# prismformore/Multi-Task-Transformer

Hardware: AMD Instinct MI355X
Metric: training images/sec (512x512, 6 tasks) (higher is better)
Workload: dtype f32(bf16x3)

## Files before the change

include/mtt_hip.h:

```cpp
#ifndef MTT_HIP_H
#define MTT_HIP_H

#include <stddef.h>
#include <stdint.h>

#ifdef __cplusplus
extern "C" {
#endif

#define MTT_ABI_VERSION 14

enum { MTT_F32 = 0, MTT_BF16 = 1, MTT_SPLIT = 2 };
enum { MTT_PREC_BF16 = 0, MTT_PREC_X3 = 1 };
enum { MTT_E_BADARG = -1, MTT_E_ALIGN = -2, MTT_E_UNSUPPORTED = -3 };

enum {
  MTT_OP_K = 0,
  MTT_OP_R = 1,
  MTT_OP_CONV_K = 2,
  MTT_OP_CONV_R = 3
};
enum { MTT_ACT_NONE = 0, MTT_ACT_GELU = 1, MTT_ACT_RELU = 2, MTT_ACT_GELU_BWD = 3, MTT_ACT_RELU_BWD = 4,
       MTT_ACT_GELU_DAUX = 5 ,
       MTT_ACT_MUL_AUX = 6    };
enum { MTT_STORE_ROWS = 0, MTT_STORE_PIXSHUF2 = 1 };
enum { MTT_GEMM_AUTO = 0,
       MTT_GEMM_GENERAL = 1           ,
       MTT_GEMM_DMA256 = 3            ,
       MTT_GEMM_DMA128 = 4            ,
       MTT_GEMM_GENERAL_EPILOGUE = 11  };
enum { MTT_ATTN_AUTO = 0, MTT_ATTN_PLAIN = 1,
       MTT_ATTN_FAST_V0 = 2 ,
       MTT_ATTN_FAST_V1 = 3  };

typedef struct {
  int32_t H, W;
  int32_t C;
  int32_t Cp;
  int32_t dil;
  int32_t flip;
} mtt_conv_geom;

typedef struct {
  const void* A; const void* B; void* D;
  int32_t M, N, K;
  int32_t a_op, b_op;
  int32_t a_dtype, b_dtype, d_dtype;
  int32_t prec;
  int64_t lda, ldb, ldd;
  int32_t a_mb; int64_t a_bs;
  int32_t d_mb; int64_t d_bs;
  int32_t batch, batch_inner;
  int64_t a_zo, a_zi, b_zo, b_zi, d_zo, d_zi;
  mtt_conv_geom conv;
  float alpha;
  const float* colscale; const float* colshift; int64_t col_zo, col_zi;
  int32_t act;
  const void* aux_in; void* aux_out; int32_t aux_dtype; int64_t ldaux; int64_t aux_zo, aux_zi;
  const float* rowscale; int32_t n_prompt;
  const float* resid; int64_t ldr; int32_t r_mb; int64_t r_bs; int64_t r_zo, r_zi;
  int32_t n_store;
  int32_t store_mode;
  int32_t ps_H, ps_W, ps_Co;
  int32_t variant;
  const void* A_lo; const void* B_lo; void* D_lo;
  float* colsum_out; float* colsum_ws;
  const float* a_scale; const float* a_shift; int32_t a_act; void* a_aux16; int64_t ld_a16;
} mtt_gemm_desc;
size_t mtt_gemm_colsum_ws_floats(const mtt_gemm_desc* d);

int mtt_abi_version(void);
size_t mtt_desc_size(int which);
int mtt_gemm(const mtt_gemm_desc* d, void* stream);
int mtt_gemm_variant(const mtt_gemm_desc* d);

typedef struct {
  const void* qkv; void* out; float* rawlog; float* lse;
  int32_t B, N, nH, T;
  int32_t dtype, prec;
  float scale;
  int32_t variant;
  const void* qkv_lo; void* out_lo;
} mtt_attn_desc;
int mtt_attn_fwd(const mtt_attn_desc* d, void* stream);
int mtt_attn_bwd(const mtt_attn_desc* d, const void* dout, const float* drawlog, void* dqkv, float* stat, void* stream);

typedef struct {
  const void* S; void* P; const void* dP; void* dS; const float* extra;
  int64_t rows, cols, ld; int32_t s_dtype, p_dtype; float scale;
  int64_t rows_per_mat; int32_t extra_rows; int64_t extra_ld;
} mtt_softmax_desc;
int mtt_softmax_fwd(const mtt_softmax_desc* d, void* stream);
int mtt_softmax_bwd(const mtt_softmax_desc* d, void* stream);

typedef struct {
  const float* x; void* y; const float* gamma; const float* beta; float* mean; float* rstd;
  const void* dy; float* dx; float* dgamma; float* dbeta;
  int64_t rows; int32_t C; int64_t ldx, ldy; int32_t y_dtype; float eps;
  const float* dx_in;
  float* ws;
  void* y_lo;
  float* y32; int64_t ldy32;
} mtt_ln_desc;
size_t mtt_layernorm_bwd_ws_floats(int64_t rows, int32_t C);
int mtt_layernorm_fwd(const mtt_ln_desc* d, void* stream);
int mtt_layernorm_bwd(const mtt_ln_desc* d, void* stream);

int mtt_patchify16(const float* img, void* cols, int B, int H, int W, int out_dtype, void* stream);

typedef struct {
  const void* q; const void* xn; float* rawchan;
  int32_t B, T, N, C, h, w, nh, nw; int32_t dtype; int64_t ldq;
  float* ws;
  const void* xn_lo;
} mtt_chanlogit_desc;
size_t mtt_chan_logits_ws_floats(const mtt_chanlogit_desc* d);
// ... 237 lines not shown
```

multi-task-transformer_amd/_lib.py:

```python
import ctypes as C
import os

import torch

_HERE = os.path.dirname(os.path.abspath(__file__))
LIB_PATH = os.path.join(_HERE, "libmtt_hip.so")

ABI_VERSION = 14
F32, BF16, SPLIT = 0, 1, 2
PREC_BF16, PREC_X3 = 0, 1
OP_K, OP_R, OP_CONV_K, OP_CONV_R = 0, 1, 2, 3
ACT_NONE, ACT_GELU, ACT_RELU, ACT_GELU_BWD, ACT_RELU_BWD, ACT_GELU_DAUX, ACT_MUL_AUX = 0, 1, 2, 3, 4, 5, 6
STORE_ROWS, STORE_PIXSHUF2 = 0, 1
GEMM_AUTO, GEMM_GENERAL, GEMM_DMA256, GEMM_DMA128, GEMM_GENERAL_EPILOGUE = 0, 1, 3, 4, 11
ATTN_AUTO, ATTN_PLAIN = 0, 1

i32, i64, f32, ptr = C.c_int32, C.c_int64, C.c_float, C.c_void_p


class ConvGeom(C.Structure):
    _fields_ = [("H", i32), ("W", i32), ("C", i32), ("Cp", i32), ("dil", i32), ("flip", i32)]


class GemmDesc(C.Structure):
    _fields_ = [
        ("A", ptr), ("B", ptr), ("D", ptr),
        ("M", i32), ("N", i32), ("K", i32),
        ("a_op", i32), ("b_op", i32),
        ("a_dtype", i32), ("b_dtype", i32), ("d_dtype", i32),
        ("prec", i32),
        ("lda", i64), ("ldb", i64), ("ldd", i64),
        ("a_mb", i32), ("a_bs", i64),
        ("d_mb", i32), ("d_bs", i64),
        ("batch", i32), ("batch_inner", i32),
        ("a_zo", i64), ("a_zi", i64), ("b_zo", i64), ("b_zi", i64), ("d_zo", i64), ("d_zi", i64),
        ("conv", ConvGeom),
        ("alpha", f32),
        ("colscale", ptr), ("colshift", ptr), ("col_zo", i64), ("col_zi", i64),
        ("act", i32),
        ("aux_in", ptr), ("aux_out", ptr), ("aux_dtype", i32), ("ldaux", i64), ("aux_zo", i64), ("aux_zi", i64),
        ("rowscale", ptr), ("n_prompt", i32),
        ("resid", ptr), ("ldr", i64), ("r_mb", i32), ("r_bs", i64), ("r_zo", i64), ("r_zi", i64),
        ("n_store", i32), ("store_mode", i32),
        ("ps_H", i32), ("ps_W", i32), ("ps_Co", i32),
        ("variant", i32),
        ("A_lo", ptr), ("B_lo", ptr), ("D_lo", ptr),
        ("colsum_out", ptr), ("colsum_ws", ptr),
        ("a_scale", ptr), ("a_shift", ptr), ("a_act", i32), ("a_aux16", ptr), ("ld_a16", i64),
    ]


class AttnDesc(C.Structure):
    _fields_ = [("qkv", ptr), ("out", ptr), ("rawlog", ptr), ("lse", ptr),
                ("B", i32), ("N", i32), ("nH", i32), ("T", i32), ("dtype", i32), ("prec", i32), ("scale", f32),
                ("variant", i32), ("qkv_lo", ptr), ("out_lo", ptr)]


class SoftmaxDesc(C.Structure):
    _fields_ = [("S", ptr), ("P", ptr), ("dP", ptr), ("dS", ptr), ("extra", ptr),
                ("rows", i64), ("cols", i64), ("ld", i64), ("s_dtype", i32), ("p_dtype", i32), ("scale", f32),
                ("rows_per_mat", i64), ("extra_rows", i32), ("extra_ld", i64)]


class LnDesc(C.Structure):
    _fields_ = [("x", ptr), ("y", ptr), ("gamma", ptr), ("beta", ptr), ("mean", ptr), ("rstd", ptr),
                ("dy", ptr), ("dx", ptr), ("dgamma", ptr), ("dbeta", ptr),
                ("rows", i64), ("C", i32), ("ldx", i64), ("ldy", i64), ("y_dtype", i32), ("eps", f32), ("dx_in", ptr), ("ws", ptr),
                ("y_lo", ptr), ("y32", ptr), ("ldy32", i64)]


class ChanLogitDesc(C.Structure):
    _fields_ = [("q", ptr), ("xn", ptr), ("rawchan", ptr),
                ("B", i32), ("T", i32), ("N", i32), ("C", i32), ("h", i32), ("w", i32), ("nh", i32), ("nw", i32),
                ("dtype", i32), ("ldq", i64), ("ws", ptr), ("xn_lo", ptr)]


class ModulateDesc(C.Structure):
    _fields_ = [("x", ptr), ("x_ld", i64), ("x_bs", i64), ("rawlog", ptr), ("rawchan", ptr), ("out", ptr),
                ("B", i32), ("T", i32), ("N", i32), ("C", i32), ("h", i32), ("w", i32), ("nh", i32), ("nw", i32),
                ("out_dtype", i32), ("hg", i32), ("out_lo", ptr)]


class CtrDesc(C.Structure):
    _fields_ = [("fea", ptr), ("out", ptr), ("wmix", ptr), ("T", i32), ("B", i32), ("rows_per_b", i64), ("ld", i64),
                ("C", i32), ("fea_dtype", i32), ("accumulate", i32), ("out_dtype", i32)]


class ResizeDesc(C.Structure):
    _fields_ = [("in_", ptr), ("out", ptr), ("B", i32), ("C", i32), ("Hin", i32), ("Win", i32), ("Hout", i32), ("Wout", i32),
                ("ld_in", i64), ("ld_out", i64), ("in_dtype", i32), ("out_dtype", i32), ("out_nchw", i32), ("accumulate", i32)]


class BnDesc(C.Structure):
    _fields_ = [("x", ptr), ("y", ptr), ("dy", ptr), ("dx", ptr),
                ("mean_out", ptr), ("m2_out", ptr), ("mean", ptr), ("rstd", ptr), ("gamma", ptr), ("beta", ptr),
                ("dsum", ptr), ("dsumxh", ptr),
                ("rows", i64), ("C", i32), ("ld", i64), ("dtype", i32), ("act", i32),
                ("Z", i32), ("x_zs", i64), ("p_zs", i64), ("g_dtype", i32)]
# ... 295 lines not shown
```

multi-task-transformer_amd/csrc/attn_bwd.hip:

```cpp
#include "mtt_device.h"
#include <type_traits>

namespace {

constexpr int HD = 64;
constexpr int KTILE = 64 * HD * 2;
constexpr float LOG2E = 1.4426950408889634f;

struct BwdP {
  const bf16_t* qkv; const bf16_t* dout; const float* stat; const float* drawlog; bf16_t* dqkv;
  int B, N, nH, T, Np; float scale;
};

__global__ __launch_bounds__(256) void attn_stat_kernel(const bf16_t* out, const bf16_t* dout, const float* lse, float* stat, int B, int N,
                                                        int nH, int Np) {
  const int C8 = nH * 8;
  const int64_t total = (int64_t)B * N * C8;
  const int64_t t = (int64_t)blockIdx.x * 256 + threadIdx.x;
  float s = 0.f;
  if (t < total) {
    const u32x4 a = *(const u32x4*)(out + t * 8), g = *(const u32x4*)(dout + t * 8);
#pragma unroll
    for (int j = 0; j < 4; ++j) s += lo_of(a[j]) * lo_of(g[j]) + hi_of(a[j]) * hi_of(g[j]);
  }
  s += __shfl_xor(s, 1, 64); s += __shfl_xor(s, 2, 64); s += __shfl_xor(s, 4, 64);
  if (t < total && (threadIdx.x & 7) == 0) {
    const int64_t tok = t / C8;
    const int h = (int)(t % C8) >> 3;
    const int b = (int)(tok / N), n = (int)(tok % N);
    float* row = stat + ((int64_t)b * nH + h) * 2 * Np;
    row[n] = s;
    row[Np + n] = lse[((int64_t)b * nH + h) * N + n] * LOG2E;
    if (n == N - 1)
      for (int k = N; k < Np; ++k) { row[k] = 0.f; row[Np + k] = 0.f; }
  }
}

MTT_DEV u32x4 perm_frag(const unsigned char* tile, int row, int ks, int lg) {
  const u32x2 lo = *(const u32x2*)(tile + lds_off(row, 4 * ks + (lg >> 1)) + (lg & 1) * 8);
  const u32x2 hi = *(const u32x2*)(tile + lds_off(row, 4 * ks + 2 + (lg >> 1)) + (lg & 1) * 8);
  return (u32x4){lo[0], lo[1], hi[0], hi[1]};
}

template <bool TR>
MTT_DEV void store_units(unsigned char* rowmajor, unsigned char* transposed, const u32x4 (&sh)[4], int kq, int rb) {
#pragma unroll
  for (int i = 0; i < 4; ++i) *(u32x4*)(rowmajor + lds_off(kq * 4 + i, rb)) = sh[i];
  if (TR) {
    u32x2 piece[8];
    transpose4x8(sh, piece);
#pragma unroll
    for (int j = 0; j < 8; ++j) *(u32x2*)(transposed + lds_off(rb * 8 + j, kq >> 1) + (kq & 1) * 8) = piece[j];
  }
}

__device__ __attribute__((aligned(32))) const unsigned g_bwd_zero_page[8] = {0u, 0u, 0u, 0u, 0u, 0u, 0u, 0u};
MTT_DEV int bwd_swz(int row) { return (((row >> 1) & 3) << 1) | ((row >> 3) & 1); }
MTT_DEV void bwd_glds16(const bf16_t* src, unsigned char* lds_wave_base) {
  __builtin_amdgcn_global_load_lds((const __attribute__((address_space(1))) void*)src,
                                   (__attribute__((address_space(3))) void*)lds_wave_base, 16, 0, 0);
}
template <int OFF>
MTT_DEV u32x2 bwd_ds_read_tr16(unsigned addr) {
  u32x2 r;
  asm volatile("ds_read_b64_tr_b16 %0, %1 offset:%2" : "=v"(r) : "v"(addr), "n"(OFF) : "memory");
  return r;
}
#define BWD_TRW(x) "+v"(x)
#define BWD_WAIT_TR8(a, b)                                                                                                              \
  asm volatile("s_waitcnt lgkmcnt(0)" : BWD_TRW(a[0]), BWD_TRW(a[1]), BWD_TRW(a[2]), BWD_TRW(a[3]), BWD_TRW(b[0]), BWD_TRW(b[1]), BWD_TRW(b[2]), BWD_TRW(b[3]) :: "memory")
#define BWD_WAIT_TR16(a, b, c, d)                                                                                                       \
  asm volatile("s_waitcnt lgkmcnt(0)" : BWD_TRW(a[0]), BWD_TRW(a[1]), BWD_TRW(a[2]), BWD_TRW(a[3]), BWD_TRW(b[0]), BWD_TRW(b[1]), BWD_TRW(b[2]), BWD_TRW(b[3]), \
               BWD_TRW(c[0]), BWD_TRW(c[1]), BWD_TRW(c[2]), BWD_TRW(c[3]), BWD_TRW(d[0]), BWD_TRW(d[1]), BWD_TRW(d[2]), BWD_TRW(d[3]) :: "memory")

template <int VER>
__global__ __launch_bounds__(256, 2) void attn_bwd_dq_kernel(const BwdP p) {
  extern __shared__ __attribute__((aligned(16))) unsigned char smem[];
  constexpr int STAGE = (VER == 2 ? 2 : 3) * KTILE;
  const int nqb = (p.N + 127) / 128;
  const int wi = xcd_remap(blockIdx.x, gridDim.x);
  const int qb = wi % nqb, bh_ = wi / nqb;
  const int h = bh_ % p.nH, b = bh_ / p.nH;
  const int N = p.N, C = p.nH * HD;
  const int tid = threadIdx.x, lane = tid & 63, wave = tid >> 6;
  const int li = lane & 15, lg = lane >> 4;
  const int64_t tok0 = (int64_t)b * N;
  const int64_t bh = (int64_t)b * p.nH + h;
  const int q0 = qb * 128 + wave * 32;
  const bool active = q0 < N;

  u32x4 qf[2][2], gf[2][2], dummy;
  float lse2[2], Dq[2];
#pragma unroll
  for (int sub = 0; sub < 2; ++sub) {
// ... 453 lines not shown
            const u32x4 ga = *(const u32x4*)(Gh + lds_off(qs * 16 + li, kh * 4 + lg));
#pragma unroll
            for (int kt = 0; kt < 2; ++kt) {
              s[q2][kt] = mfma16(qa, kf[kt][kh], s[q2][kt]);
              dp[q2][kt] = mfma16(ga, vf[kt][kh], dp[q2][kt]);
            }
          }
        }
        if (VER >= 1) __builtin_amdgcn_s_setprio(0);
        }
        u32x4 pb[2], dsb[2];
#pragma unroll
        for (int kt = 0; kt < 2; ++kt) {
          float pv[2][4], ds[2][4];
#pragma unroll
          for (int q2 = 0; q2 < 2; ++q2) {
            const float lr[4] = {L4[q2].x, L4[q2].y, L4[q2].z, L4[q2].w};
            const float dr[4] = {D4[q2].x, D4[q2].y, D4[q2].z, D4[q2].w};
#pragma unroll
            for (int r = 0; r < 4; ++r) {
              pv[q2][r] = __builtin_amdgcn_exp2f(fmaf(s[q2][kt][r], sc2, -lr[r]));
              if (!full && q0 + (2 * ks + q2) * 16 + lg * 4 + r >= N) pv[q2][r] = 0.f;
              ds[q2][r] = pv[q2][r] * (dp[q2][kt][r] - dr[r]);
            }
          }
          if (add_raw && ks == 0) {
            const int key = key0 + kt * 16 + li;
#pragma unroll
            for (int r = 0; r < 4; ++r) {
              const int q = lg * 4 + r;
              if (q < p.T && key < N) ds[0][r] += p.drawlog[(bh * p.T + q) * N + key] * inv_scale;
            }
          }
          pb[kt] = (u32x4){pack2(pv[0][0], pv[0][1]), pack2(pv[0][2], pv[0][3]), pack2(pv[1][0], pv[1][1]), pack2(pv[1][2], pv[1][3])};
          dsb[kt] = (u32x4){pack2(ds[0][0], ds[0][1]), pack2(ds[0][2], ds[0][3]), pack2(ds[1][0], ds[1][1]), pack2(ds[1][2], ds[1][3])};
        }
        if (VER >= 1) __builtin_amdgcn_s_setprio(1);
#pragma unroll
        for (int dt = 0; dt < 4; ++dt) {
          u32x4 ga, qa;
          if constexpr (VER == 2) {
            ga = (u32x4){gtl[dt][0], gtl[dt][1], gth[dt][0], gth[dt][1]};
            qa = (u32x4){qtl[dt][0], qtl[dt][1], qth[dt][0], qth[dt][1]};
          } else {
            ga = perm_frag(Gt, dt * 16 + li, ks, lg);
            qa = perm_frag(Qt, dt * 16 + li, ks, lg);
          }
#pragma unroll
          for (int kt = 0; kt < 2; ++kt) {
            dv[kt][dt] = mfma16(ga, pb[kt], dv[kt][dt]);
            dk[kt][dt] = mfma16(qa, dsb[kt], dk[kt][dt]);
          }
        }
        if (VER >= 1) __builtin_amdgcn_s_setprio(0);
      }
    }
    if (more) {
      if (VER == 2) asm volatile("s_waitcnt vmcnt(0)" ::: "memory");
      else stage_store(smem + (ST < 0 ? ((j + 1) & 1) : (1 - ST)) * STAGE);
    }
    __syncthreads();
  };
  if (VER >= 1) {
    for (int j = 0; j < nq; j += 2) {
      tile(std::integral_constant<int, 0>{}, j);
      if (j + 1 < nq) tile(std::integral_constant<int, 1>{}, j + 1);
    }
  } else {
    for (int j = 0; j < nq; ++j) tile(std::integral_constant<int, -1>{}, j);
  }
#pragma unroll
  for (int kt = 0; kt < 2; ++kt) {
    const int krow = key0 + kt * 16 + li;
    if (krow >= N) continue;
#pragma unroll
    for (int dt = 0; dt < 4; ++dt) {
      bf16_t* dst = p.dqkv + (tok0 + krow) * 3 * C + C + h * HD + dt * 16 + lg * 4;
      *(u32x2*)dst = (u32x2){pack2(dk[kt][dt][0] * p.scale, dk[kt][dt][1] * p.scale), pack2(dk[kt][dt][2] * p.scale, dk[kt][dt][3] * p.scale)};
      *(u32x2*)(dst + C) = (u32x2){pack2(dv[kt][dt][0], dv[kt][dt][1]), pack2(dv[kt][dt][2], dv[kt][dt][3])};
    }
  }
}

}

extern "C" int mtt_attn_bwd(const mtt_attn_desc* d, const void* dout, const float* drawlog, void* dqkv, float* stat, void* stream) {
  if (!d || !d->qkv || !d->out || !d->lse || !dout || !dqkv || !stat) return MTT_E_BADARG;
  if (d->B <= 0 || d->N <= 0 || d->nH <= 0 || d->T < 0 || d->T > 16) return MTT_E_BADARG;
  if (d->dtype != MTT_BF16 || d->prec != MTT_PREC_BF16) return MTT_E_UNSUPPORTED;
  if (((uintptr_t)d->qkv | (uintptr_t)dout | (uintptr_t)d->out | (uintptr_t)stat | (uintptr_t)dqkv) & 15) return MTT_E_ALIGN;
  hipStream_t s = (hipStream_t)stream;
  constexpr int smem_dq = 2 * 3 * KTILE, smem_dkv = 2 * 4 * KTILE, smem_dma = 2 * 2 * KTILE;
  static std::atomic<unsigned long long> done_dq0{0}, done_dkv0{0}, done_dq1{0}, done_dkv1{0};
  const int ver = d->variant == MTT_ATTN_FAST_V0 ? 0 : d->variant == MTT_ATTN_FAST_V1 ? 1 : 2;
  if (ver == 0) {
    if (int e = mtt_ensure_dyn_lds((const void*)attn_bwd_dq_kernel<0>, smem_dq, done_dq0)) return e;
    if (int e = mtt_ensure_dyn_lds((const void*)attn_bwd_dkv_kernel<0>, smem_dkv, done_dkv0)) return e;
  } else if (ver == 1) {
    if (int e = mtt_ensure_dyn_lds((const void*)attn_bwd_dq_kernel<1>, smem_dq, done_dq1)) return e;
    if (int e = mtt_ensure_dyn_lds((const void*)attn_bwd_dkv_kernel<1>, smem_dkv, done_dkv1)) return e;
  }
  const int Np = (d->N + 3) & ~3;
  const int64_t chunks = (int64_t)d->B * d->N * d->nH * 8;
  hipLaunchKernelGGL(attn_stat_kernel, dim3((unsigned)((chunks + 255) / 256)), dim3(256), 0, s, (const bf16_t*)d->out, (const bf16_t*)dout,
                     d->lse, stat, d->B, d->N, d->nH, Np);
  BwdP p{(const bf16_t*)d->qkv, (const bf16_t*)dout, stat, d->T > 0 ? drawlog : nullptr, (bf16_t*)dqkv, d->B, d->N, d->nH, d->T, Np, d->scale};
  dim3 grid((unsigned)(((d->N + 127) / 128) * d->nH * d->B));
  if (ver == 0) {
    hipLaunchKernelGGL(attn_bwd_dq_kernel<0>, grid, dim3(256), smem_dq, s, p);
    hipLaunchKernelGGL(attn_bwd_dkv_kernel<0>, grid, dim3(256), smem_dkv, s, p);
  } else if (ver == 1) {
    hipLaunchKernelGGL(attn_bwd_dq_kernel<1>, grid, dim3(256), smem_dq, s, p);
    hipLaunchKernelGGL(attn_bwd_dkv_kernel<1>, grid, dim3(256), smem_dkv, s, p);
  } else {
    hipLaunchKernelGGL(attn_bwd_dq_kernel<2>, grid, dim3(256), smem_dma, s, p);
    hipLaunchKernelGGL(attn_bwd_dkv_kernel<2>, grid, dim3(256), smem_dma, s, p);
  }
  return (int)hipGetLastError();
}
```

Baseline: 186.0.

## Add wide 256-row attention backward kernels with 4-stage DMA ring

Adds new dq and dkv attention-backward kernels in which each 4-wave block handles 256 query or key rows (4 sub-tiles of 16 per wave) and streams K/V or Q/dO tiles through a 4-stage global-to-LDS ring. Leftover rows are handled by a small single-wave tail kernel. This becomes the default path, and the old 128-row DMA kernel stays reachable as ROWS128. The aim is to reuse each streamed tile across more rows and to hide load latency with deeper prefetch. In exchange, each thread holds more registers, each block needs 64KB of LDS, there are fewer blocks, and tail blocks that run as one wave may be inefficient.

```diff
diff --git a/include/mtt_hip.h b/include/mtt_hip.h
--- a/include/mtt_hip.h
+++ b/include/mtt_hip.h
@@ -8,7 +8,7 @@
 extern "C" {
 #endif
 
-#define MTT_ABI_VERSION 14
+#define MTT_ABI_VERSION 15
 
 enum { MTT_F32 = 0, MTT_BF16 = 1, MTT_SPLIT = 2 };
 enum { MTT_PREC_BF16 = 0, MTT_PREC_X3 = 1 };
@@ -31,7 +31,8 @@
        MTT_GEMM_GENERAL_EPILOGUE = 11  };
 enum { MTT_ATTN_AUTO = 0, MTT_ATTN_PLAIN = 1,
        MTT_ATTN_FAST_V0 = 2 ,
-       MTT_ATTN_FAST_V1 = 3  };
+       MTT_ATTN_FAST_V1 = 3 ,
+       MTT_ATTN_ROWS128 = 4 };
 
 typedef struct {
   int32_t H, W;
diff --git a/multi-task-transformer_amd/_lib.py b/multi-task-transformer_amd/_lib.py
--- a/multi-task-transformer_amd/_lib.py
+++ b/multi-task-transformer_amd/_lib.py
@@ -6,14 +6,14 @@
 _HERE = os.path.dirname(os.path.abspath(__file__))
 LIB_PATH = os.path.join(_HERE, "libmtt_hip.so")
 
-ABI_VERSION = 14
+ABI_VERSION = 15
 F32, BF16, SPLIT = 0, 1, 2
 PREC_BF16, PREC_X3 = 0, 1
 OP_K, OP_R, OP_CONV_K, OP_CONV_R = 0, 1, 2, 3
 ACT_NONE, ACT_GELU, ACT_RELU, ACT_GELU_BWD, ACT_RELU_BWD, ACT_GELU_DAUX, ACT_MUL_AUX = 0, 1, 2, 3, 4, 5, 6
 STORE_ROWS, STORE_PIXSHUF2 = 0, 1
 GEMM_AUTO, GEMM_GENERAL, GEMM_DMA256, GEMM_DMA128, GEMM_GENERAL_EPILOGUE = 0, 1, 3, 4, 11
-ATTN_AUTO, ATTN_PLAIN = 0, 1
+ATTN_AUTO, ATTN_PLAIN, ATTN_FAST_V0, ATTN_FAST_V1, ATTN_ROWS128 = 0, 1, 2, 3, 4
 
 i32, i64, f32, ptr = C.c_int32, C.c_int64, C.c_float, C.c_void_p
 
diff --git a/multi-task-transformer_amd/csrc/attn_bwd.hip b/multi-task-transformer_amd/csrc/attn_bwd.hip
--- a/multi-task-transformer_amd/csrc/attn_bwd.hip
+++ b/multi-task-transformer_amd/csrc/attn_bwd.hip
@@ -10,6 +10,7 @@
 struct BwdP {
   const bf16_t* qkv; const bf16_t* dout; const float* stat; const float* drawlog; bf16_t* dqkv;
   int B, N, nH, T, Np; float scale;
+  int row0, nblk;
 };
 
 __global__ __launch_bounds__(256) void attn_stat_kernel(const bf16_t* out, const bf16_t* dout, const float* lse, float* stat, int B, int N,
@@ -629,6 +630,423 @@
   }
 }
 
+template <int G, int A>
+MTT_DEV void bwd_vmwait() { asm volatile("s_waitcnt vmcnt(%0)" ::"n"(A * G) : "memory"); }
+template <int G, int NST>
+MTT_DEV void bwd_ring_wait(int ahead) {
+  static_assert(NST >= 2 && NST <= 4, "ring depth");
+  if constexpr (NST >= 4) if (ahead >= 2) { bwd_vmwait<G, 2>(); return; }
+  if constexpr (NST >= 3) if (ahead >= 1) { bwd_vmwait<G, 1>(); return; }
+  bwd_vmwait<G, 0>();
+}
+MTT_DEV void bwd_ring_barrier() { asm volatile("s_waitcnt lgkmcnt(0)\n\ts_barrier" ::: "memory"); }
+
+template <int NW, int NS, int NST, int MINB>
+__global__ __launch_bounds__(NW * 64, MINB) void attn_bwd_dq_wide_kernel(const BwdP p) {
+  extern __shared__ __attribute__((aligned(16))) unsigned char smem[];
+  constexpr int STAGE = 2 * KTILE, RPW = 64 / NW, G = 2 * RPW / 8;
+  const int wi = xcd_remap(blockIdx.x, gridDim.x);
+  const int qb = wi % p.nblk, bh_ = wi / p.nblk;
+  const int h = bh_ % p.nH, b = bh_ / p.nH;
+  const int N = p.N, C = p.nH * HD;
+  const int tid = threadIdx.x, lane = tid & 63, wave = tid >> 6;
+  const int li = lane & 15, lg = lane >> 4;
+  const int64_t tok0 = (int64_t)b * N;
+  const int64_t bh = (int64_t)b * p.nH + h;
+  const int q0 = p.row0 + (qb * NW + wave) * NS * 16;
+  const bool active = q0 < N;
+
+  u32x4 qf[NS][2], gf[NS][2], dummy;
+  float lse2[NS], Dq[NS];
+#pragma unroll
+  for (int sub = 0; sub < NS; ++sub) {
+    const int qrow = q0 + sub * 16 + li;
+    const bool ok = qrow < N;
+#pragma unroll
+    for (int kh = 0; kh < 2; ++kh) {
+      Raw8<false> r;
+      load8_raw<false>(p.qkv, (tok0 + qrow) * 3 * C + h * HD + kh * 32 + lg * 8, ok, r);
+      cvt8<false, false>(ok, r, qf[sub][kh], dummy);
+      load8_raw<false>(p.dout, (tok0 + qrow) * C + h * HD + kh * 32 + lg * 8, ok, r);
+      cvt8<false, false>(ok, r, gf[sub][kh], dummy);
+    }
+    Dq[sub] = ok ? p.stat[bh * 2 * p.Np + qrow] : 0.f;
+    lse2[sub] = ok ? p.stat[bh * 2 * p.Np + p.Np + qrow] : 0.f;
+  }
+
+  int dma_off[G], dma_row[G / 2];
+  uint64_t zpage = (uint64_t)(uintptr_t)g_bwd_zero_page;
+  asm volatile("" : "+s"(zpage));
+#pragma unroll
+  for (int i = 0; i < G / 2; ++i) {
+    const int r = wave * RPW + i * 8 + (lane >> 3), pc = lane & 7;
+    dma_row[i] = r;
+    dma_off[i] = r * 3 * C + C + ((pc ^ bwd_swz(r)) & 7) * 8;
+    dma_off[G / 2 + i] = r * 3 * C + 2 * C + ((pc ^ bwd_swz(r)) & 7) * 8;
+  }
+  unsigned taddr[4];
+  const unsigned char* faddr[2];
+  {
+    const int trow = 4 * lg + (li >> 2);
+#pragma unroll
+    for (int dt = 0; dt < 4; ++dt)
+      taddr[dt] = (unsigned)(uintptr_t)smem + (unsigned)(trow * 128 + (((2 * dt + ((li & 3) >> 1)) ^ bwd_swz(trow)) & 7) * 16 + (li & 1) * 8);
+#pragma unroll
+    for (int kh = 0; kh < 2; ++kh) faddr[kh] = smem + li * 128 + (((kh * 4 + lg) ^ bwd_swz(li)) & 7) * 16;
+  }
+  auto dma_issue = [&](unsigned char* st, int kv0) {
+    const bf16_t* base = p.qkv + ((tok0 + kv0) * 3 * C + h * HD);
+    unsigned char* dK = st + wave * RPW * 128;
+    unsigned char* dV = st + KTILE + wave * RPW * 128;
+    if (kv0 + 64 <= N) {
+#pragma unroll
+      for (int i = 0; i < G / 2; ++i) bwd_glds16(base + dma_off[i], dK + i * 1024);
+#pragma unroll
+      for (int i = 0; i < G / 2; ++i) bwd_glds16(base + dma_off[G / 2 + i], dV + i * 1024);
+    } else {
+#pragma unroll
+      for (int i = 0; i < G / 2; ++i) {
+        const bool ok = kv0 + dma_row[i] < N;
+        bwd_glds16((const bf16_t*)(uintptr_t)(ok ? (uint64_t)(uintptr_t)(base + dma_off[i]) : zpage), dK + i * 1024);
+      }
+#pragma unroll
+      for (int i = 0; i < G / 2; ++i) {
+        const bool ok = kv0 + dma_row[i] < N;
+        bwd_glds16((const bf16_t*)(uintptr_t)(ok ? (uint64_t)(uintptr_t)(base + dma_off[G / 2 + i]) : zpage), dV + i * 1024);
+      }
+    }
+  };
+
+  f32x4 dq[NS][4];
+#pragma unroll
+  for (int sub = 0; sub < NS; ++sub)
+#pragma unroll
+    for (int t = 0; t < 4; ++t) dq[sub][t] = (f32x4){0.f, 0.f, 0.f, 0.f};
+  const float sc2 = p.scale * LOG2E, inv_scale = 1.0f / p.scale;
+  const bool add_raw = p.drawlog != nullptr && p.T > 0 && q0 == 0 && li < p.T;
+
+  const int nkv = (N + 63) / 64;
+#pragma unroll
+  for (int s = 0; s < NST - 1; ++s)
+    if (s < nkv) dma_issue(smem + s * STAGE, s * 64);
+  bwd_ring_wait<G, NST>(min(NST - 1, nkv) - 1);
+  bwd_ring_barrier();
+
+  auto tile = [&](auto stage_tag, int j) {
+    constexpr int ST = decltype(stage_tag)::value;
+    if (j + NST - 1 < nkv) dma_issue(smem + ((ST + NST - 1) % NST) * STAGE, (j + NST - 1) * 64);
+    const int kv0 = j * 64;
+    if (active) {
+      const bool full = kv0 + 64 <= N;
+#pragma unroll
+      for (int ks = 0; ks < 2; ++ks) {
+        if (kv0 + 32 * ks >= N) continue;
+        f32x4 s[NS][2], dp[NS][2];
+        u32x2 ktl[4], kth[4];
+        u32x4 kf[2][2], vf[2][2];
+#pragma unroll
+        for (int k2 = 0; k2 < 2; ++k2)
+#pragma unroll
+          for (int kh = 0; kh < 2; ++kh) {
+            kf[k2][kh] = *(const u32x4*)(faddr[kh] + ST * STAGE + k2 * 2048 + (ks ? 4096 : 0));
+            vf[k2][kh] = *(const u32x4*)(faddr[kh] + ST * STAGE + KTILE + k2 * 2048 + (ks ? 4096 : 0));
+          }
+        if (ks == 0) {
+#pragma unroll
+          for (int dt = 0; dt < 4; ++dt) { ktl[dt] = bwd_ds_read_tr16<ST * STAGE>(taddr[dt]); kth[dt] = bwd_ds_read_tr16<ST * STAGE + 16 * 128>(taddr[dt]); }
+        } else {
+#pragma unroll
+          for (int dt = 0; dt < 4; ++dt) { ktl[dt] = bwd_ds_read_tr16<ST * STAGE + 32 * 128>(taddr[dt]); kth[dt] = bwd_ds_read_tr16<ST * STAGE + 48 * 128>(taddr[dt]); }
+        }
+        BWD_WAIT_TR8(ktl, kth);
+        __builtin_amdgcn_s_setprio(1);
+#pragma unroll
+        for (int k2 = 0; k2 < 2; ++k2) {
+#pragma unroll
+          for (int sub = 0; sub < NS; ++sub) { s[sub][k2] = (f32x4){0.f, 0.f, 0.f, 0.f}; dp[sub][k2] = (f32x4){0.f, 0.f, 0.f, 0.f}; }
+#pragma unroll
+          for (int kh = 0; kh < 2; ++kh)
+#pragma unroll
+            for (int sub = 0; sub < NS; ++sub) {
+              s[sub][k2] = mfma16(kf[k2][kh], qf[sub][kh], s[sub][k2]);
+              dp[sub][k2] = mfma16(vf[k2][kh], gf[sub][kh], dp[sub][k2]);
+            }
+        }
+        __builtin_amdgcn_s_setprio(0);
+        u32x4 dsb[NS];
+#pragma unroll
+        for (int sub = 0; sub < NS; ++sub) {
+          float ds[2][4];
+#pragma unroll
+          for (int k2 = 0; k2 < 2; ++k2)
+#pragma unroll
+            for (int r = 0; r < 4; ++r) {
+              const float pv = __builtin_amdgcn_exp2f(fmaf(s[sub][k2][r], sc2, -lse2[sub]));
+              ds[k2][r] = pv * (dp[sub][k2][r] - Dq[sub]);
+            }
+          if (!full) {
+#pragma unroll
+            for (int k2 = 0; k2 < 2; ++k2)
+#pragma unroll
+              for (int r = 0; r < 4; ++r)
+                if (kv0 + (2 * ks + k2) * 16 + lg * 4 + r >= N) ds[k2][r] = 0.f;
+          }
+          if (sub == 0 && add_raw) {
+            const float* rl = p.drawlog + (bh * p.T + li) * N;
+#pragma unroll
+            for (int k2 = 0; k2 < 2; ++k2)
+#pragma unroll
+              for (int r = 0; r < 4; ++r) {
+                const int key = kv0 + (2 * ks + k2) * 16 + lg * 4 + r;
+                if (key < N) ds[k2][r] += rl[key] * inv_scale;
+              }
+          }
+          dsb[sub] = (u32x4){pack2(ds[0][0], ds[0][1]), pack2(ds[0][2], ds[0][3]), pack2(ds[1][0], ds[1][1]), pack2(ds[1][2], ds[1][3])};
+        }
+        __builtin_amdgcn_s_setprio(1);
+#pragma unroll
+        for (int dt = 0; dt < 4; ++dt) {
+          const u32x4 ka = (u32x4){ktl[dt][0], ktl[dt][1], kth[dt][0], kth[dt][1]};
+#pragma unroll
+          for (int sub = 0; sub < NS; ++sub) dq[sub][dt] = mfma16(ka, dsb[sub], dq[sub][dt]);
+        }
+        __builtin_amdgcn_s_setprio(0);
+      }
+    }
+    if (j + 1 < nkv) {
+      bwd_ring_wait<G, NST>(min(j + NST - 1, nkv - 1) - (j + 1));
+      bwd_ring_barrier();
+    }
+  };
+  for (int j = 0; j < nkv; j += NST) {
+    tile(std::integral_constant<int, 0>{}, j);
+    if (j + 1 < nkv) tile(std::integral_constant<int, 1>{}, j + 1);
+    if constexpr (NST > 2) if (j + 2 < nkv) tile(std::integral_constant<int, 2 % NST>{}, j + 2);
+    if constexpr (NST > 3) if (j + 3 < nkv) tile(std::integral_constant<int, 3 % NST>{}, j + 3);
+  }
+#pragma unroll
+  for (int sub = 0; sub < NS; ++sub) {
+    const int qrow = q0 + sub * 16 + li;
+    if (qrow >= N) continue;
+#pragma unroll
+    for (int dt = 0; dt < 4; ++dt)
+      *(u32x2*)(p.dqkv + (tok0 + qrow) * 3 * C + h * HD + dt * 16 + lg * 4) =
+          (u32x2){pack2(dq[sub][dt][0] * p.scale, dq[sub][dt][1] * p.scale), pack2(dq[sub][dt][2] * p.scale, dq[sub][dt][3] * p.scale)};
+  }
+}
+
+template <int NW, int NS, int NST, int MINB>
+__global__ __launch_bounds__(NW * 64, MINB) void attn_bwd_dkv_wide_kernel(const BwdP p) {
+  extern __shared__ __attribute__((aligned(16))) unsigned char smem[];
+  constexpr int STAGE = 2 * KTILE, RPW = 64 / NW, G = 2 * RPW / 8;
+  const int wi = xcd_remap(blockIdx.x, gridDim.x);
+  const int kb = wi % p.nblk, bh_ = wi / p.nblk;
+  const int h = bh_ % p.nH, b = bh_ / p.nH;
+  const int N = p.N, C = p.nH * HD;
+  const int tid = threadIdx.x, lane = tid & 63, wave = tid >> 6;
+  const int li = lane & 15, lg = lane >> 4;
+  const int64_t tok0 = (int64_t)b * N;
+  const int64_t bh = (int64_t)b * p.nH + h;
+  const int key0 = p.row0 + (kb * NW + wave) * NS * 16;
+  const bool active = key0 < N;
+
+  u32x4 kf[NS][2], vf[NS][2], dummy;
+#pragma unroll
+  for (int kt = 0; kt < NS; ++kt) {
+    const int krow = key0 + kt * 16 + li;
+    const bool ok = krow < N;
+#pragma unroll
+    for (int kh = 0; kh < 2; ++kh) {
+      Raw8<false> r;
+      load8_raw<false>(p.qkv, (tok0 + krow) * 3 * C + C + h * HD + kh * 32 + lg * 8, ok, r);
+      cvt8<false, false>(ok, r, kf[kt][kh], dummy);
+      load8_raw<false>(p.qkv, (tok0 + krow) * 3 * C + 2 * C + h * HD + kh * 32 + lg * 8, ok, r);
+      cvt8<false, false>(ok, r, vf[kt][kh], dummy);
+    }
+  }
+
+  int dma_off[G], dma_row[G / 2];
+  uint64_t zpage = (uint64_t)(uintptr_t)g_bwd_zero_page;
+  asm volatile("" : "+s"(zpage));
+#pragma unroll
+  for (int i = 0; i < G / 2; ++i) {
+    const int r = wave * RPW + i * 8 + (lane >> 3), pc = lane & 7;
+    dma_row[i] = r;
+    dma_off[i] = r * 3 * C + ((pc ^ bwd_swz(r)) & 7) * 8;
+    dma_off[G / 2 + i] = r * C + ((pc ^ bwd_swz(r)) & 7) * 8;
+  }
+  unsigned taddr[4];
+  const unsigned char* faddr[2];
+  {
+    const int trow = 4 * lg + (li >> 2);
+#pragma unroll
+    for (int dt = 0; dt < 4; ++dt)
+      taddr[dt] = (unsigned)(uintptr_t)smem + (unsigned)(trow * 128 + (((2 * dt + ((li & 3) >> 1)) ^ bwd_swz(trow)) & 7) * 16 + (li & 1) * 8);
+#pragma unroll
+    for (int kh = 0; kh < 2; ++kh) faddr[kh] = smem + li * 128 + (((kh * 4 + lg) ^ bwd_swz(li)) & 7) * 16;
+  }
+  auto dma_issue = [&](unsigned char* st, int q0) {
+    const bf16_t* baseQ = p.qkv + ((tok0 + q0) * 3 * C + h * HD);
+    const bf16_t* baseG = p.dout + ((tok0 + q0) * C + h * HD);
+    unsigned char* dQ = st + wave * RPW * 128;
+    unsigned char* dG = st + KTILE + wave * RPW * 128;
+    if (q0 + 64 <= N) {
+#pragma unroll
+      for (int i = 0; i < G / 2; ++i) bwd_glds16(baseQ + dma_off[i], dQ + i * 1024);
+#pragma unroll
+      for (int i = 0; i < G / 2; ++i) bwd_glds16(baseG + dma_off[G / 2 + i], dG + i * 1024);
+    } else {
+#pragma unroll
+      for (int i = 0; i < G / 2; ++i) {
+        const bool ok = q0 + dma_row[i] < N;
+        bwd_glds16((const bf16_t*)(uintptr_t)(ok ? (uint64_t)(uintptr_t)(baseQ + dma_off[i]) : zpage), dQ + i * 1024);
+      }
+#pragma unroll
+      for (int i = 0; i < G / 2; ++i) {
+        const bool ok = q0 + dma_row[i] < N;
+        bwd_glds16((const bf16_t*)(uintptr_t)(ok ? (uint64_t)(uintptr_t)(baseG + dma_off[G / 2 + i]) : zpage), dG + i * 1024);
+      }
+    }
+  };
+
+  f32x4 dk[NS][4], dv[NS][4];
+#pragma unroll
+  for (int kt = 0; kt < NS; ++kt)
+#pragma unroll
+    for (int t = 0; t < 4; ++t) { dk[kt][t] = (f32x4){0.f, 0.f, 0.f, 0.f}; dv[kt][t] = (f32x4){0.f, 0.f, 0.f, 0.f}; }
+  const float sc2 = p.scale * LOG2E, inv_scale = 1.0f / p.scale;
+  const float* Drow = p.stat + bh * 2 * p.Np;
+  const float* Lrow = Drow + p.Np;
+
+  const int nq = (N + 63) / 64;
+#pragma unroll
+  for (int s = 0; s < NST - 1; ++s)
+    if (s < nq) dma_issue(smem + s * STAGE, s * 64);
+  bwd_ring_wait<G, NST>(min(NST - 1, nq) - 1);
+  bwd_ring_barrier();
+
+  auto tile = [&](auto stage_tag, int j) {
+    constexpr int ST = decltype(stage_tag)::value;
+    const int q0 = j * 64;
+    float4 D4[4], L4[4];
+#pragma unroll
+    for (int qs = 0; qs < 4; ++qs) {
+      const int qr = q0 + qs * 16 + lg * 4;
+      D4[qs] = qr < p.Np ? *(const float4*)(Drow + qr) : make_float4(0.f, 0.f, 0.f, 0.f);
+      L4[qs] = qr < p.Np ? *(const float4*)(Lrow + qr) : make_float4(0.f, 0.f, 0.f, 0.f);
+    }
+    if (j + NST - 1 < nq) dma_issue(smem + ((ST + NST - 1) % NST) * STAGE, (j + NST - 1) * 64);
+    if (active) {
+      const bool full = q0 + 64 <= N;
+      const bool add_raw = p.drawlog != nullptr && j == 0 && p.T > 0;
+#pragma unroll
+      for (int ks = 0; ks < 2; ++ks) {
+        if (q0 + 32 * ks >= N) continue;
+        f32x4 s[2][NS], dp[2][NS];
+        u32x2 qtl[4], qth[4], gtl[4], gth[4];
+        u32x4 qa[2][2], ga[2][2];
+#pragma unroll
+        for (int q2 = 0; q2 < 2; ++q2)
+#pragma unroll
+          for (int kh = 0; kh < 2; ++kh) {
+            qa[q2][kh] = *(const u32x4*)(faddr[kh] + ST * STAGE + q2 * 2048 + (ks ? 4096 : 0));
+            ga[q2][kh] = *(const u32x4*)(faddr[kh] + ST * STAGE + KTILE + q2 * 2048 + (ks ? 4096 : 0));
+          }
+        if (ks == 0) {
+#pragma unroll
+          for (int dt = 0; dt < 4; ++dt) {
+            qtl[dt] = bwd_ds_read_tr16<ST * STAGE>(taddr[dt]); qth[dt] = bwd_ds_read_tr16<ST * STAGE + 16 * 128>(taddr[dt]);
+            gtl[dt] = bwd_ds_read_tr16<ST * STAGE + KTILE>(taddr[dt]); gth[dt] = bwd_ds_read_tr16<ST * STAGE + KTILE + 16 * 128>(taddr[dt]);
+          }
+        } else {
+#pragma unroll
+          for (int dt = 0; dt < 4; ++dt) {
+            qtl[dt] = bwd_ds_read_tr16<ST * STAGE + 32 * 128>(taddr[dt]); qth[dt] = bwd_ds_read_tr16<ST * STAGE + 48 * 128>(taddr[dt]);
+            gtl[dt] = bwd_ds_read_tr16<ST * STAGE + KTILE + 32 * 128>(taddr[dt]); gth[dt] = bwd_ds_read_tr16<ST * STAGE + KTILE + 48 * 128>(taddr[dt]);
+          }
+        }
+        BWD_WAIT_TR16(qtl, qth, gtl, gth);
+        __builtin_amdgcn_s_setprio(1);
+#pragma unroll
+        for (int q2 = 0; q2 < 2; ++q2) {
+#pragma unroll
+          for (int kt = 0; kt < NS; ++kt) { s[q2][kt] = (f32x4){0.f, 0.f, 0.f, 0.f}; dp[q2][kt] = (f32x4){0.f, 0.f, 0.f, 0.f}; }
+#pragma unroll
+          for (int kh = 0; kh < 2; ++kh)
+#pragma unroll
+            for (int kt = 0; kt < NS; ++kt) {
+              s[q2][kt] = mfma16(qa[q2][kh], kf[kt][kh], s[q2][kt]);
+              dp[q2][kt] = mfma16(ga[q2][kh], vf[kt][kh], dp[q2][kt]);
+            }
+        }
+        __builtin_amdgcn_s_setprio(0);
+        u32x4 pb[NS], dsb[NS];
+#pragma unroll
+        for (int kt = 0; kt < NS; ++kt) {
+          float pv[2][4], ds[2][4];
+#pragma unroll
+          for (int q2 = 0; q2 < 2; ++q2) {
+            const float4 L = L4[2 * ks + q2], D = D4[2 * ks + q2];
+            const float lr[4] = {L.x, L.y, L.z, L.w};
+            const float dr[4] = {D.x, D.y, D.z, D.w};
+#pragma unroll
+            for (int r = 0; r < 4; ++r) {
+              pv[q2][r] = __builtin_amdgcn_exp2f(fmaf(s[q2][kt][r], sc2, -lr[r]));
+              if (!full && q0 + (2 * ks + q2) * 16 + lg * 4 + r >= N) pv[q2][r] = 0.f;
+              ds[q2][r] = pv[q2][r] * (dp[q2][kt][r] - dr[r]);
+            }
+          }
+          if (add_raw && ks == 0) {
+            const int key = key0 + kt * 16 + li;
+#pragma unroll
+            for (int r = 0; r < 4; ++r) {
+              const int q = lg * 4 + r;
+              if (q < p.T && key < N) ds[0][r] += p.drawlog[(bh * p.T + q) * N + key] * inv_scale;
+            }
+          }
+          pb[kt] = (u32x4){pack2(pv[0][0], pv[0][1]), pack2(pv[0][2], pv[0][3]), pack2(pv[1][0], pv[1][1]), pack2(pv[1][2], pv[1][3])};
+          dsb[kt] = (u32x4){pack2(ds[0][0], ds[0][1]), pack2(ds[0][2], ds[0][3]), pack2(ds[1][0], ds[1][1]), pack2(ds[1][2], ds[1][3])};
+        }
+        __builtin_amdgcn_s_setprio(1);
+#pragma unroll
+        for (int dt = 0; dt < 4; ++dt) {
+          const u32x4 ga_t = (u32x4){gtl[dt][0], gtl[dt][1], gth[dt][0], gth[dt][1]};
+          const u32x4 qa_t = (u32x4){qtl[dt][0], qtl[dt][1], qth[dt][0], qth[dt][1]};
+#pragma unroll
+          for (int kt = 0; kt < NS; ++kt) {
+            dv[kt][dt] = mfma16(ga_t, pb[kt], dv[kt][dt]);
+            dk[kt][dt] = mfma16(qa_t, dsb[kt], dk[kt][dt]);
+          }
+        }
+        __builtin_amdgcn_s_setprio(0);
+      }
+    }
+    if (j + 1 < nq) {
+      bwd_ring_wait<G, NST>(min(j + NST - 1, nq - 1) - (j + 1));
+      bwd_ring_barrier();
+    }
+  };
+  for (int j = 0; j < nq; j += NST) {
+    tile(std::integral_constant<int, 0>{}, j);
+    if (j + 1 < nq) tile(std::integral_constant<int, 1>{}, j + 1);
+    if constexpr (NST > 2) if (j + 2 < nq) tile(std::integral_constant<int, 2 % NST>{}, j + 2);
+    if constexpr (NST > 3) if (j + 3 < nq) tile(std::integral_constant<int, 3 % NST>{}, j + 3);
+  }
+#pragma unroll
+  for (int kt = 0; kt < NS; ++kt) {
+    const int krow = key0 + kt * 16 + li;
+    if (krow >= N) continue;
+#pragma unroll
+    for (int dt = 0; dt < 4; ++dt) {
+      bf16_t* dst = p.dqkv + (tok0 + krow) * 3 * C + C + h * HD + dt * 16 + lg * 4;
+      *(u32x2*)dst = (u32x2){pack2(dk[kt][dt][0] * p.scale, dk[kt][dt][1] * p.scale), pack2(dk[kt][dt][2] * p.scale, dk[kt][dt][3] * p.scale)};
+      *(u32x2*)(dst + C) = (u32x2){pack2(dv[kt][dt][0], dv[kt][dt][1]), pack2(dv[kt][dt][2], dv[kt][dt][3])};
+    }
+  }
+}
+
+constexpr int WIDE_NST = 4;
+
 }
 
 extern "C" int mtt_attn_bwd(const mtt_attn_desc* d, const void* dout, const float* drawlog, void* dqkv, float* stat, void* stream) {
@@ -638,8 +1056,9 @@
   if (((uintptr_t)d->qkv | (uintptr_t)dout | (uintptr_t)d->out | (uintptr_t)stat | (uintptr_t)dqkv) & 15) return MTT_E_ALIGN;
   hipStream_t s = (hipStream_t)stream;
   constexpr int smem_dq = 2 * 3 * KTILE, smem_dkv = 2 * 4 * KTILE, smem_dma = 2 * 2 * KTILE;
+  constexpr int smem_wide = WIDE_NST * 2 * KTILE, smem_tail = 2 * 2 * KTILE;
   static std::atomic<unsigned long long> done_dq0{0}, done_dkv0{0}, done_dq1{0}, done_dkv1{0};
-  const int ver = d->variant == MTT_ATTN_FAST_V0 ? 0 : d->variant == MTT_ATTN_FAST_V1 ? 1 : 2;
+  const int ver = d->variant == MTT_ATTN_FAST_V0 ? 0 : d->variant == MTT_ATTN_FAST_V1 ? 1 : d->variant == MTT_ATTN_ROWS128 ? 2 : 3;
   if (ver == 0) {
     if (int e = mtt_ensure_dyn_lds((const void*)attn_bwd_dq_kernel<0>, smem_dq, done_dq0)) return e;
     if (int e = mtt_ensure_dyn_lds((const void*)attn_bwd_dkv_kernel<0>, smem_dkv, done_dkv0)) return e;
@@ -647,21 +1066,32 @@
     if (int e = mtt_ensure_dyn_lds((const void*)attn_bwd_dq_kernel<1>, smem_dq, done_dq1)) return e;
     if (int e = mtt_ensure_dyn_lds((const void*)attn_bwd_dkv_kernel<1>, smem_dkv, done_dkv1)) return e;
   }
+  static_assert(smem_wide <= 64 * 1024, "wide ring above the default dynamic LDS");
   const int Np = (d->N + 3) & ~3;
   const int64_t chunks = (int64_t)d->B * d->N * d->nH * 8;
   hipLaunchKernelGGL(attn_stat_kernel, dim3((unsigned)((chunks + 255) / 256)), dim3(256), 0, s, (const bf16_t*)d->out, (const bf16_t*)dout,
                      d->lse, stat, d->B, d->N, d->nH, Np);
-  BwdP p{(const bf16_t*)d->qkv, (const bf16_t*)dout, stat, d->T > 0 ? drawlog : nullptr, (bf16_t*)dqkv, d->B, d->N, d->nH, d->T, Np, d->scale};
-  dim3 grid((unsigned)(((d->N + 127) / 128) * d->nH * d->B));
+  BwdP p{(const bf16_t*)d->qkv, (const bf16_t*)dout, stat, d->T > 0 ? drawlog : nullptr, (bf16_t*)dqkv, d->B, d->N, d->nH, d->T, Np, d->scale, 0, 0};
+  const unsigned bhn = (unsigned)(d->nH * d->B);
+  dim3 grid((unsigned)((d->N + 127) / 128) * bhn);
   if (ver == 0) {
     hipLaunchKernelGGL(attn_bwd_dq_kernel<0>, grid, dim3(256), smem_dq, s, p);
     hipLaunchKernelGGL(attn_bwd_dkv_kernel<0>, grid, dim3(256), smem_dkv, s, p);
   } else if (ver == 1) {
     hipLaunchKernelGGL(attn_bwd_dq_kernel<1>, grid, dim3(256), smem_dq, s, p);
     hipLaunchKernelGGL(attn_bwd_dkv_kernel<1>, grid, dim3(256), smem_dkv, s, p);
-  } else {
+  } else if (ver == 2) {
     hipLaunchKernelGGL(attn_bwd_dq_kernel<2>, grid, dim3(256), smem_dma, s, p);
     hipLaunchKernelGGL(attn_bwd_dkv_kernel<2>, grid, dim3(256), smem_dma, s, p);
+  } else {
+    const int nfull = d->N / 256, rem = d->N - nfull * 256;
+    BwdP pm = p, pt = p;
+    pm.row0 = 0; pm.nblk = nfull;
+    pt.row0 = nfull * 256; pt.nblk = (rem + 31) / 32;
+    if (nfull) hipLaunchKernelGGL((attn_bwd_dq_wide_kernel<4, 4, WIDE_NST, 1>), dim3((unsigned)nfull * bhn), dim3(256), smem_wide, s, pm);
+    if (rem) hipLaunchKernelGGL((attn_bwd_dq_wide_kernel<1, 2, 2, 2>), dim3((unsigned)pt.nblk * bhn), dim3(64), smem_tail, s, pt);
+    if (nfull) hipLaunchKernelGGL((attn_bwd_dkv_wide_kernel<4, 4, WIDE_NST, 1>), dim3((unsigned)nfull * bhn), dim3(256), smem_wide, s, pm);
+    if (rem) hipLaunchKernelGGL((attn_bwd_dkv_wide_kernel<1, 2, 2, 2>), dim3((unsigned)pt.nblk * bhn), dim3(64), smem_tail, s, pt);
   }
   return (int)hipGetLastError();
 }
```

New measurement: 175.8, median of 2. -5.5%, worse.
